# Sukikui/PTI-LDM-VAE

Hardware: AMD Instinct MI355X
Metric: vae_train_images_per_sec_256x256 (higher is better)
Workload: dtype fp16 forward operands + activations / bf16 backward operands + gradients, fp32 accumulate; 1 GPU; config/vae_dente_no_adv.json 256x256x1 batch 32/GPU: fwd + L1 + 1e-3*KL + bwd + all-reduce + Adam (perceptual term omitted: --perceptual times it; adversarial branch inactive before epoch 6, --adv times it); global_batch=32, parallelism=dp1

## Files before the change

include/pti_vae.h:

```cpp
#ifndef PTI_VAE_H
#define PTI_VAE_H

#include <stdint.h>

#ifdef __cplusplus
extern "C" {
#endif

typedef void* pti_stream_t;

#define PTI_ABI_VERSION 5

#define PTI_OK 0
#define PTI_EINVAL (-1)
#define PTI_EUNSUPPORTED (-2)
#define PTI_ELAUNCH (-3)

#define PTI_CONV_S1 0
#define PTI_CONV_S2PAD 1
#define PTI_CONV_UP2 2
#define PTI_CONV_ZINS 3

#define PTI_PRO_NONE 0
#define PTI_PRO_GN 1
// ... 96 lines not shown
int pti_gn_bwd_blocks(int n, int hw, int c);
int pti_gn_bwd(const void* x, const void* da, const void* dres, void* dx, const int64_t* stats,
               const float* gamma, const float* beta, float* sums, float* partials, float* dgamma,
               float* dbeta, int n, int hw, int c, int groups, float eps, int silu, int x_f16,
               pti_stream_t s);
int pti_conv_gnbwd_tiles(const pti_conv_desc* d);
int pti_conv_gnbwd_chain_supported(int cin, int cout, int ksize);
int pti_conv2d_mfma_gnbwd_chain(const void* g_in, const void* x_in, int x_in_f16, const int64_t* in_stats,
                                const float* in_gamma, const float* in_sums, void* dx_in_out, const void* w_packed,
                                const void* gx, const int64_t* gstats, const float* ggamma, const float* gbeta,
                                void* dy_out, float* gsums, const pti_conv_desc* d, int silu, pti_stream_t s);
int pti_gn_affine_grads(const float* sums, float* dgamma, float* dbeta, int n, int c, pti_stream_t s);
int pti_gn_sums_finalize_affine(const float* partials, float* sums, int n, int tiles, int row_len, const float* affine_sums,
                                float* dgamma, float* dbeta, int affine_c, pti_stream_t s);
int pti_conv2d_mfma_gnbwd(const void* dy_in, const void* w_packed, const void* gx, const int64_t* gstats,
                          const float* ggamma, const float* gbeta, void* dy_out, float* gpartials,
                          const pti_conv_desc* d, int silu, pti_stream_t s);
int pti_gn_sums_finalize(const float* partials, float* sums, int n, int tiles, int row_len,
                         pti_stream_t s);
int pti_gn_bwd_apply(const void* x, const void* dy, const void* dres, void* dx, const int64_t* stats,
                     const float* gamma, const float* beta, const float* sums, float* dgamma,
                     float* dbeta, int n, int hw, int c, int groups, float eps, int x_f16,
                     pti_stream_t s);
int pti_pool2x2_sum(const void* x, void* y, int n, int h, int w, int c, pti_stream_t s);

int pti_attention_fwd(const void* qkv, void* o, float* lse2, int b, int l, int c, pti_stream_t s);
int pti_attention_bwd(const void* qkv, const void* o, const void* dout, const float* lse2,
                      float* delta, void* dqkv, int b, int l, int c, pti_stream_t s);

int pti_latent_head_fwd(const float* h, const float* eps, const float* wm, const float* bm,
                        const float* wl, const float* bl, const float* wp, const float* bp,
                        float* mu, float* sigma, float* logvar, float* zq, int b, int hw, int l,
                        pti_stream_t s);
int pti_post_quant(const float* z_nchw, const float* wp, const float* bp, float* zq_nhwc, int b,
                   int hw, int l, pti_stream_t s);
#define PTI_POST_QUANT_BWD_MAX_BLOCKS 256
#define PTI_POST_QUANT_BWD_WS_FLOATS(l) (PTI_POST_QUANT_BWD_MAX_BLOCKS * ((l) * (l) + (l)))
int pti_post_quant_bwd(const float* dzq_nhwc, const float* z_nchw, const float* wp, float* dz_nchw,
                       float* gwp, float* gbp, float* workspace, int b, int hw, int l,
                       pti_stream_t s);
#define PTI_LATENT_BWD_MAX_BLOCKS 512
#define PTI_LATENT_BWD_WS_FLOATS(l) (PTI_LATENT_BWD_MAX_BLOCKS * 3 * ((l) * (l) + (l)))
int pti_latent_head_bwd(const float* h, const float* eps, const float* wm, const float* bm,
                        const float* wl, const float* bl, const float* wp, const float* bp,
                        const float* dzq, const float* dmu, const float* dsigma, float* dh,
                        float* gwm, float* gbm, float* gwl, float* gbl, float* gwp, float* gbp,
// ... 192 lines not shown
```

pti_ldm_vae_amd/_lib.py:

```python
from __future__ import annotations

import ctypes as C
import os

_HERE = os.path.dirname(os.path.abspath(__file__))
LIB_PATH = os.environ.get("PTI_VAE_LIB") or os.path.join(_HERE, "libpti_vae_hip.so")

def env_overrides() -> dict:
    return {k: v for k, v in sorted(os.environ.items()) if k.startswith("PTI_")}


def refuse_wrong_result_env(who: str) -> None:
    bad = [k for k in os.environ if k.startswith("PTI_") and ("DIAG" in k or k == "PTI_ALLOW_WRONG_RESULTS")]
    if bad:
        raise SystemExit(f"{who}: refusing to run with wrong-result diagnostic variable(s) set: {sorted(bad)} "
                         "(timing diagnostics live in tools/diag_skip.py)")


ABI_VERSION = 5
PTI_CONV_S1, PTI_CONV_S2PAD, PTI_CONV_UP2, PTI_CONV_ZINS = 0, 1, 2, 3
PTI_PRO_NONE, PTI_PRO_GN, PTI_PRO_GN_SILU = 0, 1, 2


class ConvDesc(C.Structure):
# ... 61 lines not shown
    "pti_gn_stats": (_I, [_P, _P, _I, _I, _I, _I, _I, _P]),
    "pti_conv2d_mfma": (_I, [_P, _P, _P, _P, _P, _P, _P, _P, _P, C.POINTER(ConvDesc), _P]),
    "pti_conv2d_mfma_saveact": (_I, [_P, _P, _P, _P, _P, _P, _P, _P, _P, _P, C.POINTER(ConvDesc), _P]),
    "pti_conv2d_direct": (_I, [_P, _P, _P, _P, _P, _P, _P, C.POINTER(ConvDesc), _P]),
    "pti_wgrad_direct": (_I, [_P, _P, _P, _P, _P, _P, _P, _P, _I, _I, _I, _I, _I, _I, _I, _I, _I, _F, _I, _I,
                              C.POINTER(_I64), _I64, _I64, _I64, _P, _I64, _P]),
    "pti_conv_wgrad_workspace_bytes": (_I64, [_I, _I, _I, _I]),
    "pti_conv_wgrad_mfma": (_I, [_P, _P, _P, _P, _P, _P, _P, _P, _I64, _I, C.POINTER(ConvDesc), _P]),
    "pti_conv_wgrad_mfma_partials": (_I, [_P, _P, _P, _P, _P, _P, _I64, C.POINTER(ConvDesc), C.POINTER(_I), _P]),
    "pti_conv_wgrad_mfma_batched": (_I, [C.POINTER(WgradJob), _I, _P, _I64, _P]),
    "pti_conv_wgrad_batched_mode": (_I, [_I, _I, _I, _I, _I]),
    "pti_direct_repack": (_I, [C.POINTER(DirectRepackTable), _P]),
    "pti_conv_wgrad_reduce": (_I, [_P, _I, _P, _P, _I, C.POINTER(ConvDesc), _P]),
    "pti_gn_bwd_blocks": (_I, [_I, _I, _I]),
    "pti_gn_bwd": (_I, [_P, _P, _P, _P, _P, _P, _P, _P, _P, _P, _P, _I, _I, _I, _I, _F, _I, _I, _P]),
    "pti_conv_gnbwd_tiles": (_I, [C.POINTER(ConvDesc)]),
    "pti_gn_sums_finalize": (_I, [_P, _P, _I, _I, _I, _P]),
    "pti_conv2d_mfma_gnbwd": (_I, [_P, _P, _P, _P, _P, _P, _P, _P, C.POINTER(ConvDesc), _I, _P]),
    "pti_conv_gnbwd_chain_supported": (_I, [_I, _I, _I]),
    "pti_conv2d_mfma_gnbwd_chain": (_I, [_P, _P, _I, _P, _P, _P, _P, _P, _P, _P, _P, _P, _P, _P, C.POINTER(ConvDesc), _I, _P]),
    "pti_gn_affine_grads": (_I, [_P, _P, _P, _I, _I, _P]),
    "pti_gn_sums_finalize_affine": (_I, [_P, _P, _I, _I, _I, _P, _P, _P, _I, _P]),
    "pti_gn_bwd_apply": (_I, [_P, _P, _P, _P, _P, _P, _P, _P, _P, _P, _I, _I, _I, _I, _F, _I, _P]),
    "pti_pool2x2_sum": (_I, [_P, _P, _I, _I, _I, _I, _P]),
    "pti_attention_fwd": (_I, [_P, _P, _P, _I, _I, _I, _P]),
    "pti_attention_bwd": (_I, [_P, _P, _P, _P, _P, _P, _I, _I, _I, _P]),
    "pti_latent_head_fwd": (_I, [_P] * 12 + [_I, _I, _I, _P]),
    "pti_post_quant": (_I, [_P, _P, _P, _P, _I, _I, _I, _P]),
    "pti_post_quant_bwd": (_I, [_P, _P, _P, _P, _P, _P, _P, _I, _I, _I, _P]),
    "pti_latent_head_bwd": (_I, [_P] * 19 + [_I, _I, _I, _P]),
    "pti_vae_loss": (_I, [_P, _P, _I64, _P, _P, _I64, _I, _P, _P, _P, _P, _P, _I, _I, _F, _P]),
    "pti_ar_vae_loss": (_I, [_P, _I, _I, _I, _P, _P, _P, _I, _P, _F, _P, _P, _P, _P]),
    "pti_pd_im2col_image": (_I, [_P, _P, _I, _I, _I, _P]),
    "pti_pd_im2col": (_I, [_P, _P, _P, _I, _I, _I, _I, _I, _I, _F, _P]),
    "pti_pd_in_stats": (_I, [_P, _P, _I, _I, _I, _F, _P]),
    "pti_pd_col2im_blocks": (_I, [_I, _I, _I]),
    "pti_pd_col2im": (_I, [_P, _P, _P, _P, _P, _I, _I, _I, _I, _I, _F, _P]),
    "pti_pd_col2im_image": (_I, [_P, _P, _I, _I, _I, _F, _I, _P]),
    "pti_pd_in_bwd_apply": (_I, [_P, _P, _P, _P, _P, _I, _I, _I, _P]),
    "pti_pd_lsgan_blocks": (_I, [_I]),
    "pti_pd_lsgan": (_I, [_P, _I, _I, _I, _F, _F, _F, _P, _P, _P]),
    "pti_pd_final_fwd": (_I, [_P, _P, _P, _P, _P, _I, _I, _I, _I, _F, _P]),
    "pti_pd_final_dgrad": (_I, [_P, _P, _P, _P, _P, _P, _I, _I, _I, _I, _F, _P]),
    "pti_pd_final_wgrad_blocks": (_I, [_I, _I, _I]),
    "pti_pd_final_wgrad": (_I, [_P, _P, _P, _P, _I, _I, _I, _I, _F, _P]),
    "pti_lpips_tap_blocks": (_I, [_I, _I]),
# ... 107 lines not shown
```

pti_ldm_vae_amd/csrc/groupnorm.hip:

```cpp
#include "pti_common.h"

namespace {

__global__ __launch_bounds__(256) void gn_stats_kernel(const bf16* __restrict__ x, stat_t* __restrict__ stats,
                                                       int HW, int C, int G, int pix_per_block, int x_f16) {
  extern __shared__ stat_t sm_q[];
  stat_t* sm = sm_q;
  const int n = blockIdx.y;
  const int tid = threadIdx.x;
  const int NC = C / 8;
  const int ppi = 256 / NC;
  const int lc = tid % NC, lp = tid / NC;
  for (int i = tid; i < 2 * G; i += 256) sm[i] = 0;
  __syncthreads();
  const int p0 = blockIdx.x * pix_per_block;
  const int p1 = min(p0 + pix_per_block, HW);
  float s[8], q[8];
#pragma unroll
  for (int j = 0; j < 8; ++j) s[j] = q[j] = 0.f;
  const bf16* base = x + (size_t)n * HW * C + lc * 8;
  int p = p0 + lp;
  for (; p + 3 * ppi < p1; p += 4 * ppi) {
    u32x4 r[4];
#pragma unroll
// ... 62 lines not shown
  int bps = cdiv(2048, n);
  int ppb = cdiv(hw, bps);
  if (ppb < 16 * ppi) ppb = 16 * ppi;
  ppb = cdiv(ppb, 4 * ppi) * 4 * ppi;
  bps = cdiv(hw, ppb);
  PTI_LAUNCH(gn_stats_kernel, dim3(bps, n), dim3(256), 2 * groups * sizeof(stat_t), (hipStream_t)s,
                     (const bf16*)x, (stat_t*)stats, hw, c, groups, ppb, x_f16);
  PTI_CHECK_LAUNCH("gn_stats");
  return PTI_OK;
}

namespace {

struct GnbArgs {
  const bf16* x; const bf16* da; const bf16* dres; bf16* dx;
  const stat_t* stats; const float* gamma; const float* beta;
  float* sums;
  float* dgamma; float* dbeta;
  int HW, C, G, silu, ppb;
  float eps, inv_cnt;
  int x_f16;
  int N;
  float* part;
};

__global__ __launch_bounds__(256) void gn_bwd_reduce_kernel(GnbArgs a) {
  extern __shared__ float sm[];
  const int n = blockIdx.y, tid = threadIdx.x;
  const int NC = a.C / 8, ppi = 256 / NC, lc = tid % NC, lp = tid / NC;
  for (int i = tid; i < 8 * a.C; i += 256) sm[i] = 0.f;
  __syncthreads();
  const int cpg = a.C / a.G;
  float sc[8], sh[8], mu[8], rs[8];
#pragma unroll
  for (int j = 0; j < 8; ++j) {
    const int ch = lc * 8 + j, g = ch / cpg;
    const float sum = stat_f(a.stats, (n * a.G + g) * 2), sq = stat_f(a.stats, (n * a.G + g) * 2 + 1);
    const float mean = sum * a.inv_cnt;
    const float rstd = rsqrtf(fmaxf(sq * a.inv_cnt - mean * mean, 0.f) + a.eps);
    mu[j] = mean; rs[j] = rstd;
    sc[j] = rstd * a.gamma[ch];
    sh[j] = a.beta[ch] - mean * sc[j];
  }
  float s1[8], s2[8];
#pragma unroll
  for (int j = 0; j < 8; ++j) s1[j] = s2[j] = 0.f;
// ... 67 lines not shown
  if (i < R) {
    const float* p = part + (size_t)n * T * R + i;
    int t = w;
    for (; t + 48 < T; t += 64) {
      const float a0 = p[(size_t)t * R], a1 = p[(size_t)(t + 16) * R], a2 = p[(size_t)(t + 32) * R], a3 = p[(size_t)(t + 48) * R];
      v += (a0 + a1) + (a2 + a3);
    }
    for (; t < T; t += 16) v += p[(size_t)t * R];
  }
  red[w][lane] = v;
  __syncthreads();
  if (w == 0 && i < R) {
    float r[16];
#pragma unroll
    for (int k = 0; k < 16; ++k) r[k] = red[k][lane];
#pragma unroll
    for (int o = 8; o > 0; o >>= 1)
#pragma unroll
      for (int k = 0; k < o; ++k) r[k] += r[k + o];
    sums[(size_t)n * R + i] = r[0];
  }
}

__global__ __launch_bounds__(256) void gn_bwd_apply_kernel(GnbArgs a) {
  const int n = blockIdx.y, tid = threadIdx.x;
  const int NC = a.C / 8, ppi = 256 / NC, lc = tid % NC, lp = tid / NC;
  const int cpg = a.C / a.G;
  const int p0 = blockIdx.x * a.ppb, p1 = min(p0 + a.ppb, a.HW);
  const size_t base = (size_t)n * a.HW * a.C + lc * 8;
  constexpr int U = 4;
  u32x4 rx[U], rd[U], rr[U];
  auto load_batch = [&](int pb) {
#pragma unroll
    for (int u = 0; u < U; ++u) {
      const int p = pb + u * ppi;
      rx[u] = rd[u] = rr[u] = u32x4{0u, 0u, 0u, 0u};
      if (p < p1) {
        rx[u] = __builtin_nontemporal_load((const u32x4*)(a.x + base + (size_t)p * a.C));
        rd[u] = __builtin_nontemporal_load((const u32x4*)(a.da + base + (size_t)p * a.C));
        if (a.dres) rr[u] = __builtin_nontemporal_load((const u32x4*)(a.dres + base + (size_t)p * a.C));
      }
    }
  };
  if (p0 + lp < p1) load_batch(p0 + lp);
  float sc[8], sh[8], mu[8], rs[8], ga[8], c1[8], c2[8];
#pragma unroll
  for (int j = 0; j < 8; ++j) {
    const int ch = lc * 8 + j, g = ch / cpg;
    const float sum = stat_f(a.stats, (n * a.G + g) * 2), sq = stat_f(a.stats, (n * a.G + g) * 2 + 1);
    const float mean = sum * a.inv_cnt;
    const float rstd = rsqrtf(fmaxf(sq * a.inv_cnt - mean * mean, 0.f) + a.eps);
    mu[j] = mean; rs[j] = rstd; ga[j] = a.gamma[ch];
    sc[j] = rstd * ga[j];
    sh[j] = a.beta[ch] - mean * sc[j];
    c1[j] = c2[j] = 0.f;
    if (cpg > 8) {
      float t1 = 0.f, t2 = 0.f;
      for (int cc = g * cpg; cc < (g + 1) * cpg; ++cc) {
        const float gm = a.gamma[cc];
        t1 += gm * a.sums[((size_t)n * a.C + cc) * 2];
        t2 += gm * a.sums[((size_t)n * a.C + cc) * 2 + 1];
      }
      c1[j] = t1 * a.inv_cnt;
      c2[j] = t2 * a.inv_cnt;
    }
  }
  if (cpg <= 8) {
    float w1[8], w2[8];
#pragma unroll
    for (int j = 0; j < 8; ++j) {
      const f32x2 sv = *(const f32x2*)(a.sums + ((size_t)n * a.C + lc * 8 + j) * 2);
      w1[j] = ga[j] * sv[0];
      w2[j] = ga[j] * sv[1];
    }
#pragma unroll
    for (int j = 0; j < 8; ++j) {
      float t1 = 0.f, t2 = 0.f;
#pragma unroll
      for (int jj = 0; jj < 8; ++jj) {
        const bool same = (jj / cpg) == (j / cpg);
        t1 += same ? w1[jj] : 0.f;
        t2 += same ? w2[jj] : 0.f;
      }
      c1[j] = t1 * a.inv_cnt;
      c2[j] = t2 * a.inv_cnt;
    }
  }
  if (blockIdx.x == 0 && n == 0) {
    for (int i = tid; i < a.C; i += 256) {
      float d1 = 0.f, d2 = 0.f;
      for (int m = 0; m < a.N; ++m) {
        d1 += a.sums[((size_t)m * a.C + i) * 2];
        d2 += a.sums[((size_t)m * a.C + i) * 2 + 1];
      }
      if (a.dbeta) a.dbeta[i] += d1;
      if (a.dgamma) a.dgamma[i] += d2;
    }
  }
  for (int pb = p0 + lp; pb < p1; pb += U * ppi) {
    if (pb != p0 + lp) load_batch(pb);
#pragma unroll
    for (int u = 0; u < U; ++u) {
      const int p = pb + u * ppi;
      float fx[8], fd[8], fr[8], o[8];
      unpack8f(rx[u], fx, a.x_f16);
      unpack8(rd[u], fd);
      unpack8(rr[u], fr);
#pragma unroll
      for (int j = 0; j < 8; ++j) {
        float dy = fd[j];
        if (a.silu) dy *= dsilu_f(fx[j] * sc[j] + sh[j]);
// ... 28 lines not shown
}

}

static int gnb_min_iters() {
  static const int v = getenv("PTI_GNB_MIN_ITERS") ? atoi(getenv("PTI_GNB_MIN_ITERS")) : 8;
  return v < 1 ? 1 : v;
}
static int gn_bwd_grid(int n, int hw, int c, int* ppb_out) {
  const int ppi = 256 / (c / 8);
  int bps = cdiv(2048, n);
  int ppb = cdiv(hw, bps);
  if (ppb < gnb_min_iters() * ppi) ppb = gnb_min_iters() * ppi;
  ppb = cdiv(ppb, ppi) * ppi;
  if (ppb_out) *ppb_out = ppb;
  return cdiv(hw, ppb);
}

extern "C" int pti_gn_bwd_blocks(int n, int hw, int c) {
  if (n <= 0 || hw <= 0 || c < 8 || (c & (c - 1)) || c > 512) return 0;
  return gn_bwd_grid(n, hw, c, nullptr);
}

extern "C" int pti_gn_bwd(const void* x, const void* da, const void* dres, void* dx, const int64_t* stats,
                          const float* gamma, const float* beta, float* sums, float* partials, float* dgamma,
                          float* dbeta, int n, int hw, int c, int groups, float eps, int silu, int x_f16, pti_stream_t s) {
  if (!x || !da || !dx || !stats || !gamma || !beta || !sums || !partials) PTI_FAIL(PTI_EINVAL, "gn_bwd: null pointer");
  if (c < 8 || c > 512 || (c & (c - 1)) || groups <= 0 || c % groups) PTI_FAIL(PTI_EUNSUPPORTED, "gn_bwd: c=%d groups=%d", c, groups);
  GnbArgs a;
  a.x = (const bf16*)x; a.da = (const bf16*)da; a.dres = (const bf16*)dres; a.dx = (bf16*)dx;
  a.stats = (const stat_t*)stats; a.gamma = gamma; a.beta = beta; a.sums = sums; a.dgamma = dgamma; a.dbeta = dbeta;
  a.HW = hw; a.C = c; a.G = groups; a.silu = silu; a.eps = eps; a.x_f16 = x_f16; a.N = n;
  a.inv_cnt = 1.0f / ((float)(c / groups) * (float)hw);
  int ppb;
  const int bps = gn_bwd_grid(n, hw, c, &ppb);
  a.ppb = ppb;
  a.part = partials;
  PTI_LAUNCH(gn_bwd_reduce_kernel, dim3(bps, n), dim3(256), 8 * c * sizeof(float), (hipStream_t)s, a);
  PTI_CHECK_LAUNCH("gn_bwd_reduce");
  PTI_LAUNCH(gn_sums_finalize_kernel, dim3(cdiv(2 * c, 64), n), dim3(1024), 0, (hipStream_t)s, partials, sums,
                     bps, 2 * c, (const float*)nullptr, (float*)nullptr, (float*)nullptr, 0, 0);
  PTI_CHECK_LAUNCH("gn_sums_finalize");
  PTI_LAUNCH(gn_bwd_apply_kernel, dim3(bps, n), dim3(256), 0, (hipStream_t)s, a);
  PTI_CHECK_LAUNCH("gn_bwd_apply");
  return PTI_OK;
}

extern "C" int pti_gn_bwd_apply(const void* x, const void* dy, const void* dres, void* dx, const int64_t* stats,
                                const float* gamma, const float* beta, const float* sums, float* dgamma, float* dbeta,
                                int n, int hw, int c, int groups, float eps, int x_f16, pti_stream_t s) {
  if (!x || !dy || !dx || !stats || !gamma || !beta || !sums) PTI_FAIL(PTI_EINVAL, "gn_bwd_apply: null pointer");
  if (c < 8 || c > 2048 || (c & (c - 1)) || groups <= 0 || c % groups) PTI_FAIL(PTI_EUNSUPPORTED, "gn_bwd_apply: c=%d groups=%d", c, groups);
  GnbArgs a;
  a.x = (const bf16*)x; a.da = (const bf16*)dy; a.dres = (const bf16*)dres; a.dx = (bf16*)dx;
  a.stats = (const stat_t*)stats; a.gamma = gamma; a.beta = beta; a.sums = const_cast<float*>(sums); a.dgamma = dgamma; a.dbeta = dbeta;
  a.HW = hw; a.C = c; a.G = groups; a.silu = 0; a.eps = eps; a.x_f16 = x_f16; a.N = n;
  a.inv_cnt = 1.0f / ((float)(c / groups) * (float)hw);
  const int ppi = 256 / (c / 8);
  int bps = cdiv(2048, n);
  int ppb = cdiv(hw, bps);
  if (ppb < gnb_min_iters() * ppi) ppb = gnb_min_iters() * ppi;
  ppb = cdiv(ppb, ppi) * ppi;
  bps = cdiv(hw, ppb);
  a.ppb = ppb;
  PTI_LAUNCH(gn_bwd_apply_kernel, dim3(bps, n), dim3(256), 0, (hipStream_t)s, a);
  PTI_CHECK_LAUNCH("gn_bwd_apply");
  return PTI_OK;
}

namespace {
__global__ __launch_bounds__(256) void gn_affine_grads_kernel(const float* __restrict__ sums, float* __restrict__ dgamma,
                                                              float* __restrict__ dbeta, int n, int c) {
  const int i = blockIdx.x * 256 + threadIdx.x;
  if (i >= c) return;
  float d1 = 0.f, d2 = 0.f;
  for (int m = 0; m < n; ++m) {
    const f32x2 sv = *(const f32x2*)(sums + ((size_t)m * c + i) * 2);
    d1 += sv[0];
    d2 += sv[1];
  }
  if (dbeta) dbeta[i] += d1;
  if (dgamma) dgamma[i] += d2;
}
}

extern "C" int pti_gn_affine_grads(const float* sums, float* dgamma, float* dbeta, int n, int c, pti_stream_t s) {
  if (!sums || n <= 0 || c <= 0) PTI_FAIL(PTI_EINVAL, "gn_affine_grads: bad args");
  PTI_LAUNCH(gn_affine_grads_kernel, dim3(cdiv(c, 256)), dim3(256), 0, (hipStream_t)s, sums, dgamma, dbeta, n, c);
  PTI_CHECK_LAUNCH("gn_affine_grads");
  return PTI_OK;
// ... 30 lines not shown
```

pti_ldm_vae_amd/engine.py:

```python
from __future__ import annotations

import contextlib
import gc
import os
import warnings

import torch

from . import ops
from .models import autoencoderkl as M
from .ops import (BF16, F32, PTI_CONV_S1, PTI_CONV_S2PAD, PTI_CONV_UP2, PTI_CONV_ZINS, PTI_PRO_GN, PTI_PRO_GN_SILU,
                  PTI_PRO_NONE)


class _Act:

    __slots__ = ("t", "stats")

    def __init__(self, t, stats=None):
        self.t, self.stats = t, stats


def _empty(shape, like, dtype=BF16):
    return torch.empty(shape, dtype=dtype, device=like.device)
# ... 68 lines not shown
        y = _empty((n, ho, wo, self.cout), x.t, out_dtype or eng.act_dtype)
        st = eng.new_stats(n) if want_stats else None
        g, b = (norm.weight.data, norm.bias.data) if norm is not None else (None, None)
        ops.conv_mfma(x.t, self.wp, self.bias(), y, cout=self.cout, ksize=self.ksize, mode=self.mode, prologue=pro,
                      in_stats=x.stats if pro else None, gamma=g, beta=b, groups=eng.G, eps=eng.eps,
                      residual=residual, out_stats=st, out_groups=eng.G, act_out=act_out)
        return _Act(y, st)

    def dgrad(self, dy, *, residual=None):
        n, ho, wo, _ = dy.shape
        if self.mode == PTI_CONV_S2PAD:
            out = _empty((n, 2 * ho, 2 * wo, self.cin), dy)
            ops.conv_mfma(dy, self.wpt, None, out, cout=self.cin, ksize=3, mode=PTI_CONV_ZINS, residual=residual)
            return out
        if self.mode == PTI_CONV_UP2:
            pooled = _empty((n, ho // 2, wo // 2, self.cin), dy)
            ops.conv_mfma(dy, self.wpt, None, pooled, cout=self.cin, ksize=self.ksize, mode=PTI_CONV_S1, pool2=True)
            return pooled
        out = _empty((n, ho, wo, self.cin), dy)
        ops.conv_mfma(dy, self.wpt, None, out, cout=self.cin, ksize=self.ksize, mode=PTI_CONV_S1, residual=residual)
        return out

    def dgrad_gn(self, dy, x, norm, *, silu, dres, eng):
        g, sums = self.dgrad_gn_raw(dy, x, norm, silu=silu, eng=eng)
        return self._gn_apply(g, sums, x, norm, dres, eng)

    def _gn_apply(self, g, sums, x, norm, dres, eng):
        dx = _empty(x.t.shape, x.t)
        ops.gn_bwd_apply(x.t, g, dx, x.stats, norm.weight.data, norm.bias.data, sums,
                         norm.net.grad_view(norm.prefix + ".weight"), norm.net.grad_view(norm.prefix + ".bias"),
                         groups=eng.G, eps=eng.eps, dres=dres)
        return dx

    def dgrad_gn_raw(self, dy, x, norm, *, silu, eng):
        n, ho, wo, _ = dy.shape
        g = _empty((n, ho, wo, self.cin), dy)
        sums = eng.zeros(n * self.cin * 2)
        ops.conv_mfma_gnbwd(dy, self.wpt, x.t, x.stats, norm.weight.data, norm.bias.data, g, sums, cout=self.cin,
                            ksize=self.ksize, mode=PTI_CONV_S1, groups=eng.G, eps=eng.eps, silu=silu)
        return g, sums

    def dgrad_gn_chain(self, g_in, x_in, norm_in, sums_in, x, norm, *, silu, dres, eng):
        n, ho, wo, _ = g_in.shape
        dxin = _empty(g_in.shape, g_in)
        dyt = _empty((n, ho, wo, self.cin), g_in)
        sums = eng.zeros(n * self.cin * 2)
        ops.conv_mfma_gnbwd_chain(g_in, x_in.t, x_in.stats, norm_in.weight.data, sums_in, dxin, self.wpt, x.t, x.stats,
                                  norm.weight.data, norm.bias.data, dyt, sums, cout=self.cin, groups=eng.G, eps=eng.eps,
# ... 739 lines not shown
```

pti_ldm_vae_amd/ops.py:

```python
from __future__ import annotations

import ctypes as C
import os
from collections import namedtuple

import torch

from . import _lib as L
from ._lib import (PTI_CONV_S1, PTI_CONV_S2PAD, PTI_CONV_UP2, PTI_CONV_ZINS, PTI_PRO_GN, PTI_PRO_GN_SILU,
                   PTI_PRO_NONE, ConvDesc)

BF16 = torch.bfloat16
F16 = torch.float16
F32 = torch.float32
I64 = torch.int64
I32 = torch.int32
I16 = torch.int16
STAT_SCALE = 65536.0
ACT16 = (BF16, F16)
LATENT_BWD_MAX_BLOCKS = 512
VAE_LOSS_MAX_BLOCKS = 1024
POST_QUANT_BWD_MAX_BLOCKS = 256


# ... 361 lines not shown

def gn_bwd(x, da, dx, stats, gamma, beta, sums, dgamma, dbeta, *, groups, eps=1e-6, silu=True, dres=None):
    _chk(x, ACT16, "x", 4)
    _chk(da, BF16, "da", 4)
    _chk(dx, BF16, "dx", 4)
    n, h, w, c = x.shape
    if da.shape != x.shape or dx.shape != x.shape or (dres is not None and dres.shape != x.shape):
        raise ValueError("gn_bwd: shape mismatch")
    _chk_stats(stats, n * groups * 2, "stats")
    if sums.numel() != n * c * 2:
        raise ValueError("gn_bwd: scratch sizes")
    blocks = L.lib().pti_gn_bwd_blocks(n, h * w, c)
    if blocks <= 0:
        raise ValueError(f"gn_bwd: unsupported channel count {c}")
    part = torch.empty(n * blocks * c * 2, dtype=torch.float32, device=x.device)
    L.check(L.lib().pti_gn_bwd(_ptr(x), _ptr(da), _ptr(dres), _ptr(dx), _ptr(stats), _ptr(gamma), _ptr(beta),
                               _ptr(sums), _ptr(part), _ptr(dgamma), _ptr(dbeta), n, h * w, c, groups, eps, int(silu),
                               int(x.dtype == F16), _stream()), "pti_gn_bwd")
    return dx


def conv_mfma_gnbwd(dy_in, w_packed_t, gx, gstats, ggamma, gbeta, dy_out, gsums, *, cout, ksize=3, mode=PTI_CONV_S1,
                    groups=0, eps=1e-6, silu=True):
    _chk(dy_in, BF16, "dy_in", 4)
    _chk(gx, ACT16, "gx", 4)
    _chk(dy_out, BF16, "dy_out", 4)
    n, h, w, cin = dy_in.shape
    ho, wo = conv_out_hw(h, w, mode)
    if tuple(dy_out.shape) != (n, ho, wo, cout) or gx.shape != dy_out.shape:
        raise ValueError("conv_mfma_gnbwd: shapes")
    _chk_stats(gstats, n * groups * 2, "gstats")
    if gsums.numel() != n * cout * 2 or ggamma.numel() != cout:
        raise ValueError("conv_mfma_gnbwd: GroupNorm buffers")
    d = ConvDesc(n=n, h=h, w=w, cin=cin, ho=ho, wo=wo, cout=cout, ksize=ksize, mode=mode, groups=groups, eps=eps,
                 res_f16=int(gx.dtype == F16))
    tiles = L.lib().pti_conv_gnbwd_tiles(C.byref(d))
    if tiles <= 0:
        raise ValueError("conv_mfma_gnbwd: unsupported shape")
    part = torch.empty(n * tiles * cout * 2, dtype=torch.float32, device=dy_in.device)
    prof = KERNEL_PROFILE
    rec = None if prof is None else _prof_begin(prof)
    L.check(L.lib().pti_conv2d_mfma_gnbwd(_ptr(dy_in), _ptr(w_packed_t), _ptr(gx), _ptr(gstats), _ptr(ggamma),
                                          _ptr(gbeta), _ptr(dy_out), _ptr(part), C.byref(d), int(silu), _stream()),
            "pti_conv2d_mfma_gnbwd")
    if rec is not None:
        _prof_end(rec, 2.0 * n * ho * wo * cout * cin * ksize * ksize * (0.25 if mode == PTI_CONV_ZINS else 1.0),
                  2.0 * (dy_in.numel() + 2 * dy_out.numel()),
                  ("conv dgrad+GN bwd", cin, cout, ho, wo, ksize, "zins" if mode == PTI_CONV_ZINS else "s1", n))
    L.check(L.lib().pti_gn_sums_finalize(_ptr(part), _ptr(gsums), n, tiles, 2 * cout, _stream()), "pti_gn_sums_finalize")
    return dy_out


def gnbwd_chain_supported(cin, cout, ksize, x_dtype, groups=16):
    return (x_dtype == F16 and groups > 0 and cin % groups == 0 and cin // groups >= 8
            and bool(L.lib().pti_conv_gnbwd_chain_supported(int(cin), int(cout), int(ksize))))


def conv_mfma_gnbwd_chain(g_in, x_in, in_stats, in_gamma, in_sums, dx_in, w_packed_t, gx, gstats, ggamma, gbeta, dy_out, gsums,
                          *, cout, groups, eps=1e-6, silu=True, in_dgamma=None, in_dbeta=None):
    _chk(g_in, BF16, "g_in", 4)
    _chk(x_in, ACT16, "x_in", 4)
    _chk(dx_in, BF16, "dx_in", 4)
    _chk(gx, ACT16, "gx", 4)
    _chk(dy_out, BF16, "dy_out", 4)
    n, h, w, cin = g_in.shape
    if x_in.shape != g_in.shape or dx_in.shape != g_in.shape or tuple(dy_out.shape) != (n, h, w, cout) or gx.shape != dy_out.shape:
        raise ValueError("conv_mfma_gnbwd_chain: shapes")
    _chk_stats(in_stats, n * groups * 2, "in_stats")
    _chk_stats(gstats, n * groups * 2, "gstats")
    if in_sums.numel() != n * cin * 2 or gsums.numel() != n * cout * 2 or in_gamma.numel() != cin or ggamma.numel() != cout:
        raise ValueError("conv_mfma_gnbwd_chain: GroupNorm buffers")
    d = ConvDesc(n=n, h=h, w=w, cin=cin, ho=h, wo=w, cout=cout, ksize=3, mode=PTI_CONV_S1, groups=groups, eps=eps,
                 res_f16=int(gx.dtype == F16))
# ... 15 lines not shown
                                                    _ptr(in_dbeta), cin, _stream()), "pti_gn_sums_finalize_affine")
    else:
        L.check(L.lib().pti_gn_sums_finalize(_ptr(part), _ptr(gsums), n, tiles, 2 * cout, _stream()), "pti_gn_sums_finalize")
    return dy_out


def gn_affine_grads(sums, dgamma, dbeta, n, c):
    L.check(L.lib().pti_gn_affine_grads(_ptr(sums), _ptr(dgamma), _ptr(dbeta), int(n), int(c), _stream()), "pti_gn_affine_grads")


def gn_bwd_apply(x, dy, dx, stats, gamma, beta, sums, dgamma, dbeta, *, groups, eps=1e-6, dres=None):
    _chk(x, ACT16, "x", 4)
    _chk(dy, BF16, "dy", 4)
    _chk(dx, BF16, "dx", 4)
    n, h, w, c = x.shape
    if dy.shape != x.shape or dx.shape != x.shape or (dres is not None and dres.shape != x.shape):
        raise ValueError("gn_bwd_apply: shape mismatch")
    _chk_stats(stats, n * groups * 2, "stats")
    prof = KERNEL_PROFILE
    rec = None if prof is None else _prof_begin(prof)
    L.check(L.lib().pti_gn_bwd_apply(_ptr(x), _ptr(dy), _ptr(dres), _ptr(dx), _ptr(stats), _ptr(gamma), _ptr(beta),
                                     _ptr(sums), _ptr(dgamma), _ptr(dbeta), n, h * w, c, groups, eps,
                                     int(x.dtype == F16), _stream()), "pti_gn_bwd_apply")
    if rec is not None:
        _prof_end(rec, 8.0 * x.numel(), 2.0 * x.numel() * (4 if dres is not None else 3),
                  ("GroupNorm bwd apply", c, c, h, w, 0, "-", n))
    return dx


def pool2x2_sum(x, y):
    _chk(x, BF16, "x", 4)
    _chk(y, BF16, "y", 4)
    n, h2, w2, c = x.shape
    if tuple(y.shape) != (n, h2 // 2, w2 // 2, c) or h2 % 2 or w2 % 2:
        raise ValueError("pool2x2_sum: shapes")
    L.check(L.lib().pti_pool2x2_sum(_ptr(x), _ptr(y), n, h2 // 2, w2 // 2, c, _stream()), "pti_pool2x2_sum")
    return y


def latent_head_fwd(h, eps, wm, bm, wl, bl, wp, bp, mu, sigma, logvar, zq):
    b, hw, l = h.shape
    for t, nm in ((h, "h"), (wm, "wm"), (bm, "bm"), (wl, "wl"), (bl, "bl"), (wp, "wp"), (bp, "bp"), (mu, "mu"),
                  (sigma, "sigma"), (zq, "zq")):
        _chk(t, F32, nm)
    if mu.numel() != b * hw * l or sigma.numel() != b * hw * l or zq.numel() != b * hw * l:
        raise ValueError("latent_head_fwd: output sizes")
# ... 1509 lines not shown
```

Measured before the change: 2723 images/s.

## Fold GroupNorm backward partial-sum reduction into the apply kernel

Removes the separate gn_sums_finalize launch after the conv-dgrad+GN-bwd kernel and the GN reduce kernel. Each apply block now folds the per-tile partials for its sample into shared memory, and one extra grid row (blockIdx.y == N) accumulates the affine dgamma/dbeta grads. The fold uses a fixed summation order so results stay deterministic. In exchange, every apply block redundantly re-reads the partials, and the fold is enabled only when there are at most 16 tiles.

```diff
diff --git a/include/pti_vae.h b/include/pti_vae.h
--- a/include/pti_vae.h
+++ b/include/pti_vae.h
@@ -142,6 +142,11 @@
                      const float* gamma, const float* beta, const float* sums, float* dgamma,
                      float* dbeta, int n, int hw, int c, int groups, float eps, int x_f16,
                      pti_stream_t s);
+int pti_gn_bwd_apply_fold(const void* x, const void* dy, const void* dres, void* dx, const int64_t* stats,
+                          const float* gamma, const float* beta, const float* partials, int tiles, float* dgamma,
+                          float* dbeta, int n, int hw, int c, int groups, float eps, int x_f16,
+                          pti_stream_t s);
+int pti_gn_bwd_apply_folds(int n, int hw, int c, int tiles);
 int pti_pool2x2_sum(const void* x, void* y, int n, int h, int w, int c, pti_stream_t s);
 
 int pti_attention_fwd(const void* qkv, void* o, float* lse2, int b, int l, int c, pti_stream_t s);
diff --git a/pti_ldm_vae_amd/_lib.py b/pti_ldm_vae_amd/_lib.py
--- a/pti_ldm_vae_amd/_lib.py
+++ b/pti_ldm_vae_amd/_lib.py
@@ -107,6 +107,8 @@
     "pti_gn_affine_grads": (_I, [_P, _P, _P, _I, _I, _P]),
     "pti_gn_sums_finalize_affine": (_I, [_P, _P, _I, _I, _I, _P, _P, _P, _I, _P]),
     "pti_gn_bwd_apply": (_I, [_P, _P, _P, _P, _P, _P, _P, _P, _P, _P, _I, _I, _I, _I, _F, _I, _P]),
+    "pti_gn_bwd_apply_fold": (_I, [_P, _P, _P, _P, _P, _P, _P, _P, _I, _P, _P, _I, _I, _I, _I, _F, _I, _P]),
+    "pti_gn_bwd_apply_folds": (_I, [_I, _I, _I, _I]),
     "pti_pool2x2_sum": (_I, [_P, _P, _I, _I, _I, _I, _P]),
     "pti_attention_fwd": (_I, [_P, _P, _P, _I, _I, _I, _P]),
     "pti_attention_bwd": (_I, [_P, _P, _P, _P, _P, _P, _I, _I, _I, _P]),
diff --git a/pti_ldm_vae_amd/csrc/groupnorm.hip b/pti_ldm_vae_amd/csrc/groupnorm.hip
--- a/pti_ldm_vae_amd/csrc/groupnorm.hip
+++ b/pti_ldm_vae_amd/csrc/groupnorm.hip
@@ -108,6 +108,7 @@
   int x_f16;
   int N;
   float* part;
+  int fold, T;
 };
 
 __global__ __launch_bounds__(256) void gn_bwd_reduce_kernel(GnbArgs a) {
@@ -221,7 +222,132 @@
   }
 }
 
+__device__ __forceinline__ float gn_fold_slot(const float* __restrict__ p, int T, size_t R, int w) {
+#pragma clang fp reassociate(off)
+  float acc = 0.f;
+  int t = w;
+  if (T > w + 48) {
+    const int steps = (T - w - 49) / 64 + 1;
+    if (steps >= 2) {
+      float odd = 0.f;
+      for (int j = 0; j < (steps & ~1); j += 2, t += 128) {
+        acc = (((p[t * R] + acc) + p[(t + 16) * R]) + p[(t + 32) * R]) + p[(t + 48) * R];
+        odd = (((p[(t + 64) * R] + odd) + p[(t + 80) * R]) + p[(t + 96) * R]) + p[(t + 112) * R];
+      }
+      acc = acc + odd;
+    }
+    if (steps & 1) {
+      acc = (((p[t * R] + acc) + p[(t + 16) * R]) + p[(t + 32) * R]) + p[(t + 48) * R];
+      t += 64;
+    }
+  }
+  if (t < T) {
+    const int rows = (T - t - 1) / 16 + 1;
+    if (rows >= 2) {
+      float odd = 0.f;
+      for (int j = 0; j < (rows & ~1); j += 2, t += 32) {
+        acc = p[t * R] + acc;
+        odd = p[(t + 16) * R] + odd;
+      }
+      acc = acc + odd;
+    }
+    if (rows & 1) acc = p[t * R] + acc;
+  }
+  return acc;
+}
+__device__ __forceinline__ float gn_fold_rows(const float* __restrict__ rows, int i, int T, int R) {
+#pragma clang fp reassociate(off)
+  float r[16];
+#pragma unroll
+  for (int w = 0; w < 16; ++w) r[w] = 0.f;
+  if (T <= 64) {
+#pragma nounroll
+    for (int u = 0; 16 * u < T; ++u) {
+      float x[16];
+#pragma unroll
+      for (int w = 0; w < 16; ++w) {
+        const int t = 16 * u + w;
+        x[w] = rows[(size_t)min(t, T - 1) * R + i];
+        x[w] = t < T ? x[w] : 0.f;
+      }
+#pragma unroll
+      for (int w = 0; w < 16; ++w) r[w] = x[w] + r[w];
+    }
+  } else {
+#pragma nounroll
+    for (int w = 0; w < 16; ++w) {
+      const float v = gn_fold_slot(rows + i, T, (size_t)R, w);
+#pragma unroll
+      for (int k = 0; k < 16; ++k) r[k] = k == w ? v : r[k];
+    }
+  }
+#pragma unroll
+  for (int o = 8; o > 0; o >>= 1)
+#pragma unroll
+    for (int k = 0; k < o; ++k) r[k] += r[k + o];
+  return r[0];
+}
+
+__device__ __forceinline__ void gnb_fold_affine(const GnbArgs& a, float* red ) {
+#pragma clang fp reassociate(off)
+  const int lane = threadIdx.x & 63, w = __builtin_amdgcn_readfirstlane(threadIdx.x >> 6), R = 2 * a.C;
+  for (int i0 = blockIdx.x * 64; i0 < R; i0 += gridDim.x * 64) {
+    const int i = i0 + lane;
+    float even = 0.f, odd = 0.f, last = 0.f;
+    for (int m0 = 0; m0 < a.N; m0 += 16) {
+#pragma nounroll
+      for (int k = 0; k < 4; ++k) {
+        const int m = m0 + 4 * w + k;
+        float v = 0.f;
+        if (i < R && m < a.N) v = gn_fold_rows(a.part + (size_t)m * a.T * R, i, a.T, R);
+        red[(4 * w + k) * 64 + lane] = v;
+      }
+      __syncthreads();
+      if (w == 0)
+        for (int k = 0; k < 16 && m0 + k < a.N; k += 2) {
+          if (m0 + k + 1 < a.N) {
+            even = red[k * 64 + lane] + even;
+            odd = red[(k + 1) * 64 + lane] + odd;
+          } else {
+            last = red[k * 64 + lane];
+          }
+        }
+      __syncthreads();
+    }
+    if (w == 0 && i < R) {
+      float d = even + odd;
+      if (a.N & 1) d = last + d;
+      float* dst = (i & 1) ? a.dgamma : a.dbeta;
+      if (dst) dst[i >> 1] += d;
+    }
+  }
+}
+
+__device__ __forceinline__ void gnb_group_walk_fold(const float* tot, const float* __restrict__ gamma, int c0, int c1,
+                                                    float& t1, float& t2) {
+#pragma clang fp reassociate(off)
+  float e1 = 0.f, o1 = 0.f, e2 = 0.f, o2 = 0.f;
+  int cc = c0;
+  for (; cc + 1 < c1; cc += 2) {
+    e1 = __builtin_fmaf(tot[cc * 2], gamma[cc], e1);
+    o1 = __builtin_fmaf(tot[cc * 2 + 2], gamma[cc + 1], o1);
+    e2 = __builtin_fmaf(tot[cc * 2 + 1], gamma[cc], e2);
+    o2 = __builtin_fmaf(tot[cc * 2 + 3], gamma[cc + 1], o2);
+  }
+  t1 = e1 + o1;
+  t2 = e2 + o2;
+  if (cc < c1) {
+    t1 = __builtin_fmaf(tot[cc * 2], gamma[cc], t1);
+    t2 = __builtin_fmaf(tot[cc * 2 + 1], gamma[cc], t2);
+  }
+}
+
 __global__ __launch_bounds__(256) void gn_bwd_apply_kernel(GnbArgs a) {
+  extern __shared__ float fold_sm[];
+  if (blockIdx.y == a.N) {
+    gnb_fold_affine(a, fold_sm);
+    return;
+  }
   const int n = blockIdx.y, tid = threadIdx.x;
   const int NC = a.C / 8, ppi = 256 / NC, lc = tid % NC, lp = tid / NC;
   const int cpg = a.C / a.G;
@@ -242,6 +368,11 @@
     }
   };
   if (p0 + lp < p1) load_batch(p0 + lp);
+  if (a.fold) {
+    const int R = 2 * a.C;
+    for (int i = tid; i < R; i += 256) fold_sm[i] = gn_fold_rows(a.part + (size_t)n * a.T * R, i, a.T, R);
+    if (cpg > 8) __syncthreads();
+  }
   float sc[8], sh[8], mu[8], rs[8], ga[8], c1[8], c2[8];
 #pragma unroll
   for (int j = 0; j < 8; ++j) {
@@ -255,6 +386,8 @@
     c1[j] = c2[j] = 0.f;
     if (cpg > 8) {
       float t1 = 0.f, t2 = 0.f;
+      if (a.fold) gnb_group_walk_fold(fold_sm, a.gamma, g * cpg, (g + 1) * cpg, t1, t2);
+      else
       for (int cc = g * cpg; cc < (g + 1) * cpg; ++cc) {
         const float gm = a.gamma[cc];
         t1 += gm * a.sums[((size_t)n * a.C + cc) * 2];
@@ -265,10 +398,12 @@
     }
   }
   if (cpg <= 8) {
+    if (a.fold) __syncthreads();
     float w1[8], w2[8];
 #pragma unroll
     for (int j = 0; j < 8; ++j) {
-      const f32x2 sv = *(const f32x2*)(a.sums + ((size_t)n * a.C + lc * 8 + j) * 2);
+      const f32x2 sv = a.fold ? *(const f32x2*)(fold_sm + (lc * 8 + j) * 2)
+                              : *(const f32x2*)(a.sums + ((size_t)n * a.C + lc * 8 + j) * 2);
       w1[j] = ga[j] * sv[0];
       w2[j] = ga[j] * sv[1];
     }
@@ -285,7 +420,7 @@
       c2[j] = t2 * a.inv_cnt;
     }
   }
-  if (blockIdx.x == 0 && n == 0) {
+  if (blockIdx.x == 0 && n == 0 && !a.fold) {
     for (int i = tid; i < a.C; i += 256) {
       float d1 = 0.f, d2 = 0.f;
       for (int m = 0; m < a.N; ++m) {
@@ -360,6 +495,23 @@
   return gn_bwd_grid(n, hw, c, nullptr);
 }
 
+static bool gnb_fold_enabled() {
+  const char* e = getenv("PTI_GNB_FOLD");
+  return !e || atoi(e) != 0;
+}
+
+extern "C" int pti_gn_bwd_apply_folds(int n, int hw, int c, int tiles) {
+  if (n <= 0 || hw <= 0 || tiles <= 0 || c < 8 || c > 2048 || (c & (c - 1))) return 0;
+  return gnb_fold_enabled() && tiles <= 16;
+}
+
+static void gnb_launch_apply(GnbArgs& a, int bps, int n, int c, hipStream_t s) {
+  if (a.fold)
+    PTI_LAUNCH(gn_bwd_apply_kernel, dim3(bps, n + 1), dim3(256), (2 * c > 1024 ? 2 * c : 1024) * sizeof(float), s, a);
+  else
+    PTI_LAUNCH(gn_bwd_apply_kernel, dim3(bps, n), dim3(256), 0, s, a);
+}
+
 extern "C" int pti_gn_bwd(const void* x, const void* da, const void* dres, void* dx, const int64_t* stats,
                           const float* gamma, const float* beta, float* sums, float* partials, float* dgamma,
                           float* dbeta, int n, int hw, int c, int groups, float eps, int silu, int x_f16, pti_stream_t s) {
@@ -374,36 +526,52 @@
   const int bps = gn_bwd_grid(n, hw, c, &ppb);
   a.ppb = ppb;
   a.part = partials;
+  a.T = bps;
+  a.fold = pti_gn_bwd_apply_folds(n, hw, c, bps);
   PTI_LAUNCH(gn_bwd_reduce_kernel, dim3(bps, n), dim3(256), 8 * c * sizeof(float), (hipStream_t)s, a);
   PTI_CHECK_LAUNCH("gn_bwd_reduce");
-  PTI_LAUNCH(gn_sums_finalize_kernel, dim3(cdiv(2 * c, 64), n), dim3(1024), 0, (hipStream_t)s, partials, sums,
-                     bps, 2 * c, (const float*)nullptr, (float*)nullptr, (float*)nullptr, 0, 0);
-  PTI_CHECK_LAUNCH("gn_sums_finalize");
-  PTI_LAUNCH(gn_bwd_apply_kernel, dim3(bps, n), dim3(256), 0, (hipStream_t)s, a);
+  if (!a.fold) {
+    PTI_LAUNCH(gn_sums_finalize_kernel, dim3(cdiv(2 * c, 64), n), dim3(1024), 0, (hipStream_t)s, partials, sums,
+                       bps, 2 * c, (const float*)nullptr, (float*)nullptr, (float*)nullptr, 0, 0);
+    PTI_CHECK_LAUNCH("gn_sums_finalize");
+  }
+  gnb_launch_apply(a, bps, n, c, (hipStream_t)s);
   PTI_CHECK_LAUNCH("gn_bwd_apply");
   return PTI_OK;
 }
 
-extern "C" int pti_gn_bwd_apply(const void* x, const void* dy, const void* dres, void* dx, const int64_t* stats,
-                                const float* gamma, const float* beta, const float* sums, float* dgamma, float* dbeta,
-                                int n, int hw, int c, int groups, float eps, int x_f16, pti_stream_t s) {
-  if (!x || !dy || !dx || !stats || !gamma || !beta || !sums) PTI_FAIL(PTI_EINVAL, "gn_bwd_apply: null pointer");
-  if (c < 8 || c > 2048 || (c & (c - 1)) || groups <= 0 || c % groups) PTI_FAIL(PTI_EUNSUPPORTED, "gn_bwd_apply: c=%d groups=%d", c, groups);
+static int gnb_apply(const char* who, const void* x, const void* dy, const void* dres, void* dx, const int64_t* stats,
+                     const float* gamma, const float* beta, const float* sums, const float* partials, int tiles,
+                     float* dgamma, float* dbeta, int n, int hw, int c, int groups, float eps, int x_f16, pti_stream_t s) {
+  if (!x || !dy || !dx || !stats || !gamma || !beta || (!sums && !partials)) PTI_FAIL(PTI_EINVAL, "%s: null pointer", who);
+  if (n <= 0 || hw <= 0 || (partials && tiles <= 0)) PTI_FAIL(PTI_EINVAL, "%s: n=%d hw=%d tiles=%d", who, n, hw, tiles);
+  if (c < 8 || c > 2048 || (c & (c - 1)) || groups <= 0 || c % groups) PTI_FAIL(PTI_EUNSUPPORTED, "%s: c=%d groups=%d", who, c, groups);
   GnbArgs a;
   a.x = (const bf16*)x; a.da = (const bf16*)dy; a.dres = (const bf16*)dres; a.dx = (bf16*)dx;
   a.stats = (const stat_t*)stats; a.gamma = gamma; a.beta = beta; a.sums = const_cast<float*>(sums); a.dgamma = dgamma; a.dbeta = dbeta;
   a.HW = hw; a.C = c; a.G = groups; a.silu = 0; a.eps = eps; a.x_f16 = x_f16; a.N = n;
   a.inv_cnt = 1.0f / ((float)(c / groups) * (float)hw);
-  const int ppi = 256 / (c / 8);
-  int bps = cdiv(2048, n);
-  int ppb = cdiv(hw, bps);
-  if (ppb < gnb_min_iters() * ppi) ppb = gnb_min_iters() * ppi;
-  ppb = cdiv(ppb, ppi) * ppi;
-  bps = cdiv(hw, ppb);
+  a.part = const_cast<float*>(partials); a.T = tiles; a.fold = partials != nullptr;
+  int ppb;
+  const int bps = gn_bwd_grid(n, hw, c, &ppb);
   a.ppb = ppb;
-  PTI_LAUNCH(gn_bwd_apply_kernel, dim3(bps, n), dim3(256), 0, (hipStream_t)s, a);
-  PTI_CHECK_LAUNCH("gn_bwd_apply");
+  gnb_launch_apply(a, bps, n, c, (hipStream_t)s);
+  PTI_CHECK_LAUNCH(who);
   return PTI_OK;
+}
+extern "C" int pti_gn_bwd_apply(const void* x, const void* dy, const void* dres, void* dx, const int64_t* stats,
+                                const float* gamma, const float* beta, const float* sums, float* dgamma, float* dbeta,
+                                int n, int hw, int c, int groups, float eps, int x_f16, pti_stream_t s) {
+  if (!sums) PTI_FAIL(PTI_EINVAL, "gn_bwd_apply: null pointer");
+  return gnb_apply("gn_bwd_apply", x, dy, dres, dx, stats, gamma, beta, sums, nullptr, 0, dgamma, dbeta, n, hw, c, groups, eps,
+                   x_f16, s);
+}
+extern "C" int pti_gn_bwd_apply_fold(const void* x, const void* dy, const void* dres, void* dx, const int64_t* stats,
+                                     const float* gamma, const float* beta, const float* partials, int tiles, float* dgamma,
+                                     float* dbeta, int n, int hw, int c, int groups, float eps, int x_f16, pti_stream_t s) {
+  if (!partials) PTI_FAIL(PTI_EINVAL, "gn_bwd_apply_fold: null pointer");
+  return gnb_apply("gn_bwd_apply_fold", x, dy, dres, dx, stats, gamma, beta, nullptr, partials, tiles, dgamma, dbeta, n, hw, c,
+                   groups, eps, x_f16, s);
 }
 
 namespace {
diff --git a/pti_ldm_vae_amd/engine.py b/pti_ldm_vae_amd/engine.py
--- a/pti_ldm_vae_amd/engine.py
+++ b/pti_ldm_vae_amd/engine.py
@@ -114,8 +114,19 @@
         return out
 
     def dgrad_gn(self, dy, x, norm, *, silu, dres, eng):
-        g, sums = self.dgrad_gn_raw(dy, x, norm, silu=silu, eng=eng)
-        return self._gn_apply(g, sums, x, norm, dres, eng)
+        if not ops.conv_mfma_gnbwd_folds(dy, cout=self.cin, ksize=self.ksize):
+            g, sums = self.dgrad_gn_raw(dy, x, norm, silu=silu, eng=eng)
+            return self._gn_apply(g, sums, x, norm, dres, eng)
+        n, ho, wo, _ = dy.shape
+        g = _empty((n, ho, wo, self.cin), dy)
+        _, part, tiles = ops.conv_mfma_gnbwd_parts(dy, self.wpt, x.t, x.stats, norm.weight.data, norm.bias.data, g,
+                                                   cout=self.cin, ksize=self.ksize, mode=PTI_CONV_S1, groups=eng.G,
+                                                   eps=eng.eps, silu=silu)
+        dx = _empty(x.t.shape, x.t)
+        ops.gn_bwd_apply_fold(x.t, g, dx, x.stats, norm.weight.data, norm.bias.data, part, tiles,
+                              norm.net.grad_view(norm.prefix + ".weight"), norm.net.grad_view(norm.prefix + ".bias"),
+                              groups=eng.G, eps=eng.eps, dres=dres)
+        return dx
 
     def _gn_apply(self, g, sums, x, norm, dres, eng):
         dx = _empty(x.t.shape, x.t)
diff --git a/pti_ldm_vae_amd/ops.py b/pti_ldm_vae_amd/ops.py
--- a/pti_ldm_vae_amd/ops.py
+++ b/pti_ldm_vae_amd/ops.py
@@ -407,6 +407,28 @@
 
 def conv_mfma_gnbwd(dy_in, w_packed_t, gx, gstats, ggamma, gbeta, dy_out, gsums, *, cout, ksize=3, mode=PTI_CONV_S1,
                     groups=0, eps=1e-6, silu=True):
+    part, tiles = _conv_mfma_gnbwd(dy_in, w_packed_t, gx, gstats, ggamma, gbeta, dy_out, gsums, cout, ksize, mode, groups, eps,
+                                   silu)
+    L.check(L.lib().pti_gn_sums_finalize(_ptr(part), _ptr(gsums), dy_in.shape[0], tiles, 2 * cout, _stream()),
+            "pti_gn_sums_finalize")
+    return dy_out
+
+
+def conv_mfma_gnbwd_parts(dy_in, w_packed_t, gx, gstats, ggamma, gbeta, dy_out, *, cout, ksize=3, mode=PTI_CONV_S1,
+                          groups=0, eps=1e-6, silu=True):
+    part, tiles = _conv_mfma_gnbwd(dy_in, w_packed_t, gx, gstats, ggamma, gbeta, dy_out, None, cout, ksize, mode, groups, eps,
+                                   silu)
+    return dy_out, part, tiles
+
+
+def conv_mfma_gnbwd_folds(dy_in, *, cout, ksize=3, mode=PTI_CONV_S1):
+    n, h, w, cin = dy_in.shape
+    ho, wo = conv_out_hw(h, w, mode)
+    d = ConvDesc(n=n, h=h, w=w, cin=cin, ho=ho, wo=wo, cout=cout, ksize=ksize, mode=mode)
+    return bool(L.lib().pti_gn_bwd_apply_folds(n, ho * wo, cout, L.lib().pti_conv_gnbwd_tiles(C.byref(d))))
+
+
+def _conv_mfma_gnbwd(dy_in, w_packed_t, gx, gstats, ggamma, gbeta, dy_out, gsums, cout, ksize, mode, groups, eps, silu):
     _chk(dy_in, BF16, "dy_in", 4)
     _chk(gx, ACT16, "gx", 4)
     _chk(dy_out, BF16, "dy_out", 4)
@@ -415,7 +437,7 @@
     if tuple(dy_out.shape) != (n, ho, wo, cout) or gx.shape != dy_out.shape:
         raise ValueError("conv_mfma_gnbwd: shapes")
     _chk_stats(gstats, n * groups * 2, "gstats")
-    if gsums.numel() != n * cout * 2 or ggamma.numel() != cout:
+    if (gsums is not None and gsums.numel() != n * cout * 2) or ggamma.numel() != cout:
         raise ValueError("conv_mfma_gnbwd: GroupNorm buffers")
     d = ConvDesc(n=n, h=h, w=w, cin=cin, ho=ho, wo=wo, cout=cout, ksize=ksize, mode=mode, groups=groups, eps=eps,
                  res_f16=int(gx.dtype == F16))
@@ -432,8 +454,7 @@
         _prof_end(rec, 2.0 * n * ho * wo * cout * cin * ksize * ksize * (0.25 if mode == PTI_CONV_ZINS else 1.0),
                   2.0 * (dy_in.numel() + 2 * dy_out.numel()),
                   ("conv dgrad+GN bwd", cin, cout, ho, wo, ksize, "zins" if mode == PTI_CONV_ZINS else "s1", n))
-    L.check(L.lib().pti_gn_sums_finalize(_ptr(part), _ptr(gsums), n, tiles, 2 * cout, _stream()), "pti_gn_sums_finalize")
-    return dy_out
+    return part, tiles
 
 
 def gnbwd_chain_supported(cin, cout, ksize, x_dtype, groups=16):
@@ -495,6 +516,31 @@
     L.check(L.lib().pti_gn_bwd_apply(_ptr(x), _ptr(dy), _ptr(dres), _ptr(dx), _ptr(stats), _ptr(gamma), _ptr(beta),
                                      _ptr(sums), _ptr(dgamma), _ptr(dbeta), n, h * w, c, groups, eps,
                                      int(x.dtype == F16), _stream()), "pti_gn_bwd_apply")
+    if rec is not None:
+        _prof_end(rec, 8.0 * x.numel(), 2.0 * x.numel() * (4 if dres is not None else 3),
+                  ("GroupNorm bwd apply", c, c, h, w, 0, "-", n))
+    return dx
+
+
+def gn_bwd_apply_fold(x, dy, dx, stats, gamma, beta, part, tiles, dgamma, dbeta, *, groups, eps=1e-6, dres=None):
+    _chk(x, ACT16, "x", 4)
+    _chk(dy, BF16, "dy", 4)
+    _chk(dx, BF16, "dx", 4)
+    _chk(part, F32, "part")
+    n, h, w, c = x.shape
+    if dy.shape != x.shape or dx.shape != x.shape or (dres is not None and dres.shape != x.shape):
+        raise ValueError("gn_bwd_apply_fold: shape mismatch")
+    if tiles <= 0 or part.numel() != n * tiles * c * 2 or gamma.numel() != c or beta.numel() != c:
+        raise ValueError("gn_bwd_apply_fold: partials / GroupNorm buffers")
+    for name, t in (("dgamma", dgamma), ("dbeta", dbeta)):
+        if t is not None and t.numel() != c:
+            raise ValueError(f"gn_bwd_apply_fold: {name} must hold {c} floats")
+    _chk_stats(stats, n * groups * 2, "stats")
+    prof = KERNEL_PROFILE
+    rec = None if prof is None else _prof_begin(prof)
+    L.check(L.lib().pti_gn_bwd_apply_fold(_ptr(x), _ptr(dy), _ptr(dres), _ptr(dx), _ptr(stats), _ptr(gamma), _ptr(beta),
+                                          _ptr(part), int(tiles), _ptr(dgamma), _ptr(dbeta), n, h * w, c, groups, eps,
+                                          int(x.dtype == F16), _stream()), "pti_gn_bwd_apply_fold")
     if rec is not None:
         _prof_end(rec, 8.0 * x.numel(), 2.0 * x.numel() * (4 if dres is not None else 3),
                   ("GroupNorm bwd apply", c, c, h, w, 0, "-", n))
```

Measured after the change: 2738 images/s (median of 6 runs). Within noise of the previous version (+0.6%).
